# Skylarking/MARL

Hardware: AMD Instinct MI355X
Metric: env_steps_per_sec (higher is better)
Workload: dtype f32 (bf16x6 split products, fp32 accumulate)

## Files before the change

include/marl_hip.h:

```cpp
#ifndef MARL_HIP_H
#define MARL_HIP_H
#include <stddef.h>
#ifdef __cplusplus
extern "C" {
#endif

typedef struct {
  const float* p0; long ld0; int k0;
  const float* p1; long ld1; int k1;
  const int* idx; int nhot; int hot_w;
  int nid;
  const float* m0; long ldm0;
  long rpe0, bs0, off0;
  long rpei, bsi, offi;
  const int* emap0;
} marl_src_t;

typedef struct {
  int groups;
  long gs_x0, gs_x1, gs_w, gs_b, gs_y, gs_m0;
} marl_group_t;

typedef struct {
  const float *fc1_w, *fc1_b;
// ... 18 lines not shown
                          int N, int O, int A, int last_action, int reuse_network, int cu_budget,
                          float* gi_out, const float* gi_in, void* stream);
int marl_agent_unroll_reuse_supported(int B, int T, int N, int O, int A, int cu_budget);

typedef struct {
  float *w_ih, *w_hh;
  float *b_ih, *b_hh;
  float *fc2_w, *fc2_b;
} marl_agent_grads_t;

size_t marl_agent_bwd_workspace(int B, int N, int A);
int marl_agent_unroll_bwd(const marl_agent_weights_t* w, const float* dq, const int* dq_idx,
                          const float* dq_val, const int* dq_idx2, const float* dq_val2, int dq_gdiv, const float* dhs,
                          const float* saved, const float* hs, float* dxp, float* dh0,
                          const marl_agent_grads_t* g, float* ws, size_t ws_bytes,
                          int B, int T, int N, int A, void* stream);

int marl_q_gather(const float* q, const int* idx, const float* avail, float mask_val, float* out,
                  long rows, int A, void* stream);
int marl_q_masked_max(const float* q, const float* avail, float mask_val, float* out_max, int* out_arg,
                      long rows, int A, void* stream);
int marl_q_double_select(const float* q_sel, const float* q_val, const float* avail, float mask_val,
                         float* out_val, int* out_arg, long rows, int A, void* stream);
int marl_q_scatter(float* dq, const int* idx1, const float* g1, const int* idx2, const float* g2,
                   long rows, int A, int gdiv, void* stream);
int marl_vec_add(const float* a, const float* b, float* out, long n, void* stream);
int marl_agent_sum(const float* in, long ld_in, float* out, long ld_out, long rows, int N, int D, void* stream);
int marl_agent_bcast(const float* in, long ld_in, float* out, long ld_out, long rows, int N, int D, int accumulate,
                     void* stream);

int marl_qmix_mix_fwd(const float* hy, long ldh, const float* b2, const float* w22, const float* b22, const float* q,
                      float* q_tot, long rows, int N, int E, void* stream);
int marl_qmix_mix_bwd(const float* hy, long ldh, const float* q, const float* dq_tot, const float* w22, float* dhy,
                      float* db2, float* dq, long rows, int N, int E, void* stream);
int marl_qmix_tail_fwd(const marl_src_t* s, long rows, int S, const float* Wb1, long ldb1, const float* bb1, const float* Wh,
                       long ldwh, const float* bh, float* hy, long ldhy, int c_b1, int c_h, void* stream);

typedef struct {
  const float *w1, *w1_b;
  const float *b1, *b1_b;
  const float *w2, *w2_b;
  const float *h, *h_b;
  const float *b2_w, *b2_b;
} marl_qmix_weights_t;
int marl_qmix_fused_supported(int N, int S, int E);
size_t marl_qmix_fused_workspace(long rows, int N, int S);
// ... 261 lines not shown
```

marl_amd/_lib.py:

```python
from __future__ import annotations

import ctypes as C
import os

_HERE = os.path.dirname(os.path.abspath(__file__))
LIB_PATH = os.environ.get("MARL_HIP_LIB") or os.path.join(_HERE, "libmarl_hip.so")

c_float_p = C.c_void_p
c_int_p = C.c_void_p


class MarlSrc(C.Structure):
    _fields_ = [("p0", C.c_void_p), ("ld0", C.c_long), ("k0", C.c_int),
                ("p1", C.c_void_p), ("ld1", C.c_long), ("k1", C.c_int),
                ("idx", C.c_void_p), ("nhot", C.c_int), ("hot_w", C.c_int),
                ("nid", C.c_int),
                ("m0", C.c_void_p), ("ldm0", C.c_long),
                ("rpe0", C.c_long), ("bs0", C.c_long), ("off0", C.c_long),
                ("rpei", C.c_long), ("bsi", C.c_long), ("offi", C.c_long),
                ("emap0", C.c_void_p)]


class MarlGroup(C.Structure):
    _fields_ = [("groups", C.c_int), ("gs_x0", C.c_long), ("gs_x1", C.c_long), ("gs_w", C.c_long),
# ... 67 lines not shown
WW, WG = C.POINTER(MarlWorldWeights), C.POINTER(MarlWorldGrads)
MW, MG = C.POINTER(MarlMaicWeights), C.POINTER(MarlMaicGrads)
MIW, MIG = C.POINTER(MarlMaicInfer), C.POINTER(MarlMaicInferGrads)

SIGNATURES = {
    "marl_linear": (I, [SRC, P, L, I, P, P, L, I, I, I, I, F, GRP, P]),
    "marl_linear_wgrad": (I, [P, L, P, L, SRC, P, L, P, I, I, I, I, GRP, P, SZ, P]),
    "marl_linear_wgrad_workspace": (SZ, [I, I, I, I]),
    "marl_wgrad_slabs": (I, [I]),
    "marl_agent_unroll_fwd": (I, [AW, P, L, I, P, L, I, P, P, P, P, P, P, P, I, I, I, I, I, I, I, I, P, P, P]),
    "marl_agent_unroll_reuse_supported": (I, [I, I, I, I, I, I]),
    "marl_agent_unroll_x6_supported": (I, [I, I, I, I, I, I, I]),
    "marl_agent_unroll_x6_plain_r6": (I, [I, I, I, I, I, I, I, I]),
    "marl_agent_unroll_fwd_x6": (I, [AW, P, L, I, P, L, I, P, P, P, P, P, P, P, I, I, I, I, I, I, I, I, P, P, P]),
    "marl_agent_bwd_workspace": (SZ, [I, I, I]),
    "marl_agent_unroll_bwd_x6_supported": (I, [I, I, I, I, I]),
    "marl_agent_bwd_x6_workspace": (SZ, [I, I, I]),
    "marl_agent_unroll_bwd_x6": (I, [AW, P, P, P, P, I, P, P, P, P, AG, P, SZ, I, I, I, I, P]),
    "marl_agent_unroll_bwd": (I, [AW, P, P, P, P, P, I, P, P, P, P, P, AG, P, SZ, I, I, I, I, P]),
    "marl_replay_gather": (I, [P, I, I, I, I] + [P] * 17 + [P]),
    "marl_q_gather": (I, [P, P, P, F, P, L, I, P]),
    "marl_q_masked_max": (I, [P, P, F, P, P, L, I, P]),
    "marl_q_double_select": (I, [P, P, P, F, P, P, L, I, P]),
    "marl_q_scatter": (I, [P, P, P, P, P, L, I, I, P]),
    "marl_vec_add": (I, [P, P, P, L, P]),
    "marl_agent_sum": (I, [P, L, P, L, L, I, I, P]),
    "marl_agent_bcast": (I, [P, L, P, L, L, I, I, I, P]),
    "marl_qmix_mix_fwd": (I, [P, L, P, P, P, P, P, L, I, I, P]),
    "marl_qmix_mix_bwd": (I, [P, L, P, P, P, P, P, P, L, I, I, P]),
    "marl_qmix_tail_fwd": (I, [SRC, L, I, P, L, P, P, L, P, P, L, I, I, P]),
    "marl_qmix_fused_supported": (I, [I, I, I]),
    "marl_qmix_fused_workspace": (SZ, [L, I, I]),
    "marl_qmix_fused_fwd": (I, [QW, SRC, P, P, L, I, I, I, P]),
    "marl_qmix_fused_bwd": (I, [QW, SRC, P, P, P, QW, P, SZ, L, I, I, I, P]),
    "marl_qmix_fused_loss_bwd": (I, [QW, SRC, P, P, P, P, P, F, P, P, QW, P, P, SZ, L, I, I, I, P]),
    "marl_qmix_fused_fwd_x6": (I, [QW, SRC, P, P, L, I, I, I, P]),
    "marl_qmix_fused_bwd_x6": (I, [QW, SRC, P, P, P, QW, P, SZ, L, I, I, I, P]),
    "marl_qmix_fused_loss_bwd_x6": (I, [QW, SRC, P, P, P, P, P, F, P, P, QW, P, P, SZ, L, I, I, I, P]),
    "marl_qmix_wide_supported": (I, [I, I, I]),
    "marl_qmix_wide_workspace": (SZ, [L, I, I, I]),
    "marl_qmix_wide_fwd_kernel": (C.c_char_p, [L, I, I, I]),
    "marl_qmix_wide_fwd": (I, [QW, SRC, P, P, P, SZ, L, I, I, I, I, P]),
    "marl_qmix_wide_bwd": (I, [QW, SRC, P, P, P, QW, P, SZ, L, I, I, I, I, P]),
    "marl_qmix_wide_loss_bwd": (I, [QW, SRC, P, P, P, P, P, F, P, P, QW, P, P, SZ, L, I, I, I, I, P]),
    "marl_mlp3_supported": (I, [SRC, I, I, I, I, I]),
    "marl_mlp3_fwd": (I, [M3, SRC, P, L, L, L, I, I, I, P]),
# ... 96 lines not shown
```

marl_amd/algorithm/common.py:

```python
from __future__ import annotations

import copy
import numbers
import os
import warnings
import weakref

import numpy as np
import torch

from .. import ops, experiments
from ..hostutil import FlatParams, DeviceBatch, AsyncInt, require_cuda
from ..network.mixer import x6_mode
from ..rollout import EpisodeBatch

MASK_BIG = -9999999.0
MASK_QTRAN_EVAL = -999999.0
N_STATS = 4


class FlatView:

    def __init__(self, flat, params, start):
        self.params = list(params)
# ... 142 lines not shown
        self._td_dbg = {}
        self.max_episode_len = args.episode_limit
        self.gamma = args.gamma
        self.lr = args.lr
        self.model_dir = args.model_dir + '/' + args.alg + '/' + args.map
        self.args = args
        self.device = require_cuda(name)

        self.eval_net = mac
        self.eval_net.cuda()
        self.target_net = copy.deepcopy(mac)

    def _ready(self, needs_avail):
        args = self.args
        self.optimizer = FusedOptimizer(self._flat, args.optimizer, self.lr, args.grad_norm_clip)
        self._buf = Scratch()
        self.reducer = GradReducer()
        self.pair = PairedUnroll(x6=x6_mode(args))
        self.loss_readback = LossReadback(args)
        self.graphs = GraphedUpdate.from_args(args) if self.replay_graphs else None
        self.needs_avail = needs_avail
        self.last_stats = None
        self.sync_replicas()

    def _update_targets(self):
        self.target_net.agent._flat.flat.copy_(self.eval_net.agent._flat.flat)
        if self.mixer is not None and self.mixer._flat.n:
            self.target_mixer._flat.flat.copy_(self.mixer._flat.flat)

    def _g(self, name, shape, dt=torch.float32):
        return self._buf.get(name, shape, self.device, dt)

    def _td_inputs(self, db, q_next_tot):
        lam = self.td_lambda = td_lambda_of(self.args)
        if lam is None:
            self._td_dbg = {}
            return db.r, self.gamma
        G = self._g("td_ret", (db.B * db.T,))
        ops.td_lambda_returns(q_next_tot, db.r, db.term, db.padded, self.gamma, lam, G, db.B, db.T)
        self._td_dbg = {"td_targets": G}
        return G, 0.0

    def get_max_episode_len(self, batch):
        T = DeviceBatch.first_terminated_len(torch.as_tensor(np.asarray(batch['terminated'])), self.args.episode_limit)
        for key in batch.keys():
            batch[key] = batch[key][:, :T]
# ... 8 lines not shown
            self._full_len_streak = self._full_len_streak + 1 if full else 0
            return db
        db, pending = DeviceBatch.from_record_begin(rec, self.args, reducer=self.reducer, index=index, small=small)
        self.max_episode_len = db.T
        self._forward_backward(db)
        T = pending()
        if T == db.T:
            return None
        self._full_len_streak = 0
        return DeviceBatch.from_record(rec, self.args, T=T, index=index, small=small)

    def train(self, batch, train_step):
        ring = batch.ring if isinstance(batch, EpisodeBatch) else None
        if self.graphs is not None and ring is not None and self.graphs.run(self, ring, batch.index):
            db = None
        elif isinstance(batch, DeviceBatch):
            db = batch
        elif ring is not None:
            prep = self.graphs.prepared if self.graphs is not None else None
            if prep is not None:
                self.graphs.prepared = None
                db = DeviceBatch.from_record(ring, self.args, T=prep[1], index=batch.index, small=prep[0])
            else:
                small = ring.select_small(batch.index, avail_cur=self.needs_avail)
                db = self._device_batch(ring, batch.index, small)
        elif isinstance(batch, EpisodeBatch) and batch.record is not None:
            db = self._device_batch(batch.record, None, None)
        else:
            T = None
            if self.reducer.enabled:
                T = DeviceBatch.first_terminated_len(torch.as_tensor(np.asarray(batch['terminated'])),
                                                     self.args.episode_limit, reducer=self.reducer)
            db = DeviceBatch.from_dict(batch, self.args, self.device, T=T)
        if db is not None:
            self.max_episode_len = db.T
            self._forward_backward(db)
        return self._finish_update(train_step)

    def _loss_fn(self):
        return lambda s: s[0] / s[1]

    def _finish_update(self, train_step):
        self.reducer.allreduce_(self._flat.gradx)
        stats = self._flat.stats
        self.optimizer.step(den=stats[self.den_slot:self.den_slot + 1])
        if train_step > 0 and train_step % self.args.target_update_cycle == 0:
            self._update_targets()
# ... 182 lines not shown
    SCHEDULE_ARGS = ("gemm_mode", "mixer_dtype", "mixer_wgrad_dtype", "double_q", "no_loss_fold", "lazy_loss", "gamma",
                     "two_hyper_layers", "last_action", "reuse_network", "td_lambda")

    @staticmethod
    def _schedule_key(args):
        return (experiments.generation,) + tuple(repr(getattr(args, k, None)) for k in GraphedUpdate.SCHEDULE_ARGS)

    def run(self, learner, ring, index):
        self.prepared = None
        if self.disabled:
            return False
        args = learner.args
        if self.auto and int(index.numel()) > self.AUTO_MAX_EPISODES:
            return False
        if ring.T != args.episode_limit or int(index.numel()) != int(args.batch_size):
            return False
        key = (id(ring), int(index.numel()), ring.T)
        e = self.entries.get(key)
        if e is not None and e["ring"]() is not ring:
            e = None
        dev = ring.obs.device
        if e is None:
            idx = index.to(device=dev, dtype=torch.long).clone()
            small = ring.select_small(idx, avail_cur=getattr(learner, "needs_avail", False))
            db = DeviceBatch.from_record(ring, args, T=min(ring.T, args.episode_limit), index=idx, small=small)
            fused = getattr(small, "avail_next", None) is not None and db.T == ring.T
            e = self.entries[key] = dict(ring=weakref.ref(ring), idx=idx, small=small, db=db, calls=0, graph=None, streak=0,
                                         fused=fused, avail_next=None if fused else db.avail_next.clone(),
                                         u_act=None if fused else db.u_act.clone())
            if not fused:
                db.avail_next, db.u_act = e["avail_next"], e["u_act"]
            e["T"] = db.T
        idx, small, db = e["idx"], e["small"], e["db"]
        idx.copy_(index)
        db.o_map.copy_(idx)
        ring.select_small(idx, out=small)
        if e["graph"] is not None and (e["ws_gen"] != ops.WS.gen or e["sched_key"] != self._schedule_key(args)):
            e["graph"], e["ws_keep"], e["calls"] = None, None, 0
        pending = None
        term = small.term
        if e["graph"] is not None and e["streak"] >= 2 and term.is_cuda and term.dtype == torch.float32 and term.shape[0] > 0:
            out = ops.first_terminated_len(term, args.episode_limit)
            r = learner.reducer
            if r is not None and r.enabled:
                r.dist.all_reduce(out, op=r.dist.ReduceOp.MAX, group=r.group)
            pending = AsyncInt(out)
            T = e["T"]
        else:
            T = DeviceBatch.first_terminated_len(term, args.episode_limit, reducer=learner.reducer)
# ... 42 lines not shown
```

marl_amd/algorithm/q_learner.py:

```python
from __future__ import annotations

import copy

import numpy as np
import torch

from .. import ops, experiments
from ..hostutil import flatten_module
from ..network.mixer import VDNMixer, QMixMixer, DMAQer
from .common import MASK_BIG, LearnerParams, FlatView, Learner, agent_backward


class QLearner(Learner):
    def __init__(self, mac, args):
        self._begin(mac, args, "QLearner")
        if args.alg == 'vdn':
            self.mixer = VDNMixer(args)
        elif args.alg == 'qmix':
            self.mixer = QMixMixer(args)
        elif args.alg == 'qplex':
            self.mixer = DMAQer(args)
        else:
            raise ValueError("Mixer {} not recognised.".format(args.alg))
        self.target_mixer = copy.deepcopy(self.mixer)
# ... 30 lines not shown
        if keep_hs:
            hs, hs_tgt = g("hs", (B, T, N, H)), g("hs_tgt", (B, T, N, H))
            hs_en = g("hs_en", (B, T, N, H)) if a.double_q else None
        (oc, oc_bs, oc_t0), (on, on_bs, on_t0) = db.o_cur, db.o_next

        emap = getattr(db, 'o_map', None)
        cont, gi = None, None
        if a.double_q:
            shifted = on is oc and on_bs == oc_bs and on_t0 == oc_t0 + 1
            split = self.pair.chain_split(B * N, T, a.obs_shape)
            if shifted and ((self.eval_net.unroll_x6(B, T, oc) and experiments.get("fwd_xs") != 0) or
                            ops.agent_unroll_reuse_supported(B, T, N, a.obs_shape, A, split[0] if split else 256)):
                gi = g("gi", ops.saved_shape(T, B, N, planes=3))
            cont = lambda cu: self.eval_net.unroll(on, on_bs, on_t0, db.u_fed, db.u_bs, 0, B, T, q_en, hs_en, h_scr, None, h0=h_last,
                                                   ep_len=db.ep_len, ep_map=emap, cu_budget=cu, gi_in=gi)
        self.pair.run_chain(B * N, T, a.obs_shape,
                            lambda cu: self.eval_net.unroll(oc, oc_bs, oc_t0, db.u_fed, db.u_bs, -1, B, T, q_evals, hs, h_last, saved,
                                                            h0=None, ep_len=db.ep_len, ep_map=emap, cu_budget=cu, gi_out=gi),
                            cont,
                            lambda cu: self.target_net.unroll(on, on_bs, on_t0, db.u_fed, db.u_bs, 0, B, T, q_tgt, hs_tgt, None, None,
                                                              h0=None, ep_len=db.ep_len, ep_map=emap, cu_budget=cu))
        return q_evals, q_en, q_tgt, saved, (hs, hs_en, hs_tgt)

    def _select(self, db, q_evals, q_en, q_tgt):
        R, A, g = db.B * db.T * db.N, db.A, self._g
        q_chosen, q_tgt_chosen = g("q_chosen", (R,)), g("q_tgt_chosen", (R,))
        ops.q_gather(q_evals, db.u_act.reshape(-1), q_chosen, R, A)
        cur_max = None
        if self.args.double_q:
            cur_max = g("cur_max", (R,), torch.int32)
            ops.q_double_select(q_en, q_tgt, db.avail_next, MASK_BIG, q_tgt_chosen, cur_max, R, A)
        else:
            ops.q_masked_max(q_tgt, db.avail_next, MASK_BIG, q_tgt_chosen, None, R, A)
        return q_chosen, q_tgt_chosen, cur_max

    def _mix(self, db, q_evals, q_tgt, q_chosen, q_tgt_chosen, cur_max):
        a, g = self.args, self._g
        N, BT, A = db.N, db.B * db.T, db.A
        R = BT * N
        ctx, fold = {}, False
        qc, qtc = q_chosen.view(BT, N), q_tgt_chosen.view(BT, N)
        if a.alg == 'qplex':
            max_q = g("max_q", (R,))
            ops.q_masked_max(q_evals, db.avail, MASK_BIG, max_q, None, R, A)
            v_tot, a_tot = self.mixer.hip_forward(qc, db.s, BT, u_idx=db.u_taken.reshape(-1), max_q=max_q.view(BT, N), ctx=ctx)
            q_tot = g("q_tot", (BT,))
            ops.vec_add(v_tot, a_tot, q_tot, BT)
            if a.double_q:
                tgt_max = g("tgt_max", (R,))
                ops.q_masked_max(q_tgt, db.avail_next, MASK_BIG, tgt_max, None, R, A)
                vt, at = self.target_mixer.hip_forward(qtc, db.s_next, BT, u_idx=cur_max, max_q=tgt_max.view(BT, N), tag="t")
                q_tot_tgt = g("q_tot_tgt", (BT,))
                ops.vec_add(vt, at, q_tot_tgt, BT)
            else:
# ... 51 lines not shown
```

marl_amd/csrc/mixers.hip:

```cpp
#include "common.h"
#include "sums.h"
#include "../../include/marl_hip.h"

namespace {

constexpr int TPB = 256;
static_assert(TPB == SUMS_TPB, "the loss kernels launch sums.h's workgroup size");
inline int nblk(long n, int cap = 65535 * 16) {
  long b = (n + TPB - 1) / TPB;
  if (b > cap) b = cap;
  if (b < 1) b = 1;
  return (int)b;
}

__global__ void q_gather_kernel(const float* q, const int* idx, const float* avail, float mask_val, float* out,
                                long rows, int A) {
  for (long r = (long)blockIdx.x * TPB + threadIdx.x; r < rows; r += (long)gridDim.x * TPB) {
    const int a = idx[r];
    float v = 0.f;
    if (a >= 0) v = (avail && avail[r * A + a] == 0.f) ? mask_val : q[r * A + a];
    out[r] = v;
  }
}

__global__ void q_masked_max_kernel(const float* q, const float* avail, float mask_val, float* out_max,
                                    int* out_arg, long rows, int A) {
  for (long r = (long)blockIdx.x * TPB + threadIdx.x; r < rows; r += (long)gridDim.x * TPB) {
    float best = 0.f;
    int arg = 0;
    for (int a = 0; a < A; ++a) {
      float v = q[r * A + a];
      if (avail && avail[r * A + a] == 0.f) v = mask_val;
      if (a == 0 || v > best) { best = v; arg = a; }
    }
    if (out_max) out_max[r] = best;
    if (out_arg) out_arg[r] = arg;
  }
}

constexpr int DS_ROWS = 64;
__global__ __launch_bounds__(256) void q_double_select_kernel(const float* q_sel, const float* q_val, const float* avail,
                                                              float mask_val, float* out_val, int* out_arg, long rows, int A, int vec) {
  extern __shared__ __attribute__((aligned(16))) float ds_smem[];
  const int lane = threadIdx.x & 63, wave = threadIdx.x >> 6;
  const int TS = (DS_ROWS * A + 3) & ~3;
  float* Sq = ds_smem + (size_t)wave * 3 * TS;
  float* Sv = Sq + TS;
  float* Sa = Sv + TS;
  const long tiles = (rows + DS_ROWS - 1) / DS_ROWS;
  for (long tile = (long)blockIdx.x * 4 + wave; tile < tiles; tile += (long)gridDim.x * 4) {
    const long r0 = tile * DS_ROWS;
    const int n = (int)((rows - r0 < DS_ROWS ? rows - r0 : DS_ROWS) * A);
    const float* gq = q_sel + r0 * A;
    const float* gv = q_val + r0 * A;
    const float* ga = avail ? avail + r0 * A : nullptr;
    const int n4 = vec ? n >> 2 : 0;
    for (int e = lane; e < n4; e += 64) {
      reinterpret_cast<f32x4*>(Sq)[e] = reinterpret_cast<const f32x4*>(gq)[e];
      reinterpret_cast<f32x4*>(Sv)[e] = reinterpret_cast<const f32x4*>(gv)[e];
      reinterpret_cast<f32x4*>(Sa)[e] = ga ? reinterpret_cast<const f32x4*>(ga)[e] : (f32x4){1.f, 1.f, 1.f, 1.f};
    }
    for (int e = 4 * n4 + lane; e < n; e += 64) {
      Sq[e] = gq[e]; Sv[e] = gv[e]; Sa[e] = ga ? ga[e] : 1.f;
    }
    __builtin_amdgcn_s_waitcnt(0xC07F);
    const long r = r0 + lane;
    if (r < rows) {
      float best = 0.f; int arg = 0;
      for (int a = 0; a < A; ++a) {
        float v = Sq[lane * A + a];
        if (Sa[lane * A + a] == 0.f) v = mask_val;
        if (a == 0 || v > best) { best = v; arg = a; }
      }
      out_val[r] = Sa[lane * A + arg] == 0.f ? mask_val : Sv[lane * A + arg];
      if (out_arg) out_arg[r] = arg;
    }
  }
}

__global__ void q_double_select_rows_kernel(const float* q_sel, const float* q_val, const float* avail, float mask_val,
                                            float* out_val, int* out_arg, long rows, int A) {
  for (long r = (long)blockIdx.x * TPB + threadIdx.x; r < rows; r += (long)gridDim.x * TPB) {
    float best = 0.f;
    int arg = 0;
    for (int a = 0; a < A; ++a) {
      float v = q_sel[r * A + a];
      if (avail && avail[r * A + a] == 0.f) v = mask_val;
      if (a == 0 || v > best) { best = v; arg = a; }
    }
    out_val[r] = (avail && avail[r * A + arg] == 0.f) ? mask_val : q_val[r * A + arg];
    if (out_arg) out_arg[r] = arg;
  }
}

__global__ __launch_bounds__(256) void q_masked_max_tiled_kernel(const float* q, const float* avail, float mask_val, float* out_max,
                                                                 int* out_arg, long rows, int A) {
  extern __shared__ __attribute__((aligned(16))) float ds_smem[];
  const int lane = threadIdx.x & 63, wave = threadIdx.x >> 6;
  const int TS = (DS_ROWS * A + 3) & ~3;
  float* Sq = ds_smem + (size_t)wave * 2 * TS;
  float* Sa = Sq + TS;
  const long tiles = (rows + DS_ROWS - 1) / DS_ROWS;
  for (long tile = (long)blockIdx.x * 4 + wave; tile < tiles; tile += (long)gridDim.x * 4) {
    const long r0 = tile * DS_ROWS;
    const int n = (int)((rows - r0 < DS_ROWS ? rows - r0 : DS_ROWS) * A);
    const float* gq = q + r0 * A;
    const float* ga = avail ? avail + r0 * A : nullptr;
    const int n4 = n >> 2;
    for (int e = lane; e < n4; e += 64) {
      reinterpret_cast<f32x4*>(Sq)[e] = reinterpret_cast<const f32x4*>(gq)[e];
      reinterpret_cast<f32x4*>(Sa)[e] = ga ? reinterpret_cast<const f32x4*>(ga)[e] : (f32x4){1.f, 1.f, 1.f, 1.f};
    }
    for (int e = 4 * n4 + lane; e < n; e += 64) { Sq[e] = gq[e]; Sa[e] = ga ? ga[e] : 1.f; }
// ... 370 lines not shown
  MARL_CHECK_LAUNCH();
  return 0;
}

extern "C" int marl_q_masked_max(const float* q, const float* avail, float mask_val, float* out_max, int* out_arg,
                                 long rows, int A, void* stream) {
  if (rows <= 0) return 0;
  const size_t lds = (size_t)4 * 2 * ((DS_ROWS * A + 3) & ~3) * sizeof(float);
  if (((reinterpret_cast<uintptr_t>(q) | reinterpret_cast<uintptr_t>(avail)) & 15) == 0 && lds <= 64 * 1024 && rows >= 4096) {
    const long tiles = (rows + DS_ROWS - 1) / DS_ROWS;
    long nb = (tiles + 3) / 4;
    if (nb > 2048) nb = 2048;
    hipLaunchKernelGGL(q_masked_max_tiled_kernel, dim3((unsigned)nb), dim3(256), lds, (hipStream_t)stream, q, avail, mask_val,
                       out_max, out_arg, rows, A);
    MARL_CHECK_LAUNCH();
    return 0;
  }
  hipLaunchKernelGGL(q_masked_max_kernel, dim3(nblk(rows)), dim3(TPB), 0, (hipStream_t)stream, q, avail, mask_val,
                     out_max, out_arg, rows, A);
  MARL_CHECK_LAUNCH();
  return 0;
}

extern "C" int marl_q_double_select(const float* q_sel, const float* q_val, const float* avail, float mask_val,
                                    float* out_val, int* out_arg, long rows, int A, void* stream) {
  if (rows <= 0) return 0;
  const long tiles = (rows + DS_ROWS - 1) / DS_ROWS;
  long nb = (tiles + 3) / 4;
  if (nb > 2048) nb = 2048;
  const size_t lds = (size_t)4 * 3 * ((DS_ROWS * A + 3) & ~3) * sizeof(float);
  if (lds > 64 * 1024) {
    hipLaunchKernelGGL(q_double_select_rows_kernel, dim3(nblk(rows)), dim3(TPB), 0, (hipStream_t)stream, q_sel, q_val, avail,
                       mask_val, out_val, out_arg, rows, A);
    MARL_CHECK_LAUNCH();
    return 0;
  }
  const int vec = ((reinterpret_cast<uintptr_t>(q_sel) | reinterpret_cast<uintptr_t>(q_val) | reinterpret_cast<uintptr_t>(avail)) & 15) == 0;
  hipLaunchKernelGGL(q_double_select_kernel, dim3((unsigned)nb), dim3(256), lds, (hipStream_t)stream, q_sel, q_val, avail,
                     mask_val, out_val, out_arg, rows, A, vec);
  MARL_CHECK_LAUNCH();
  return 0;
}

extern "C" int marl_q_scatter(float* dq, const int* idx1, const float* g1, const int* idx2, const float* g2,
                              long rows, int A, int gdiv, void* stream) {
  if (rows <= 0) return 0;
  hipLaunchKernelGGL(q_scatter_kernel, dim3(nblk(rows)), dim3(TPB), 0, (hipStream_t)stream, dq, idx1, g1, idx2, g2,
                     rows, A, gdiv < 1 ? 1 : gdiv);
  MARL_CHECK_LAUNCH();
  return 0;
}

extern "C" int marl_vec_add(const float* a, const float* b, float* out, long n, void* stream) {
  if (n <= 0) return 0;
  hipLaunchKernelGGL(vec_add_kernel, dim3(nblk(n, 4096)), dim3(TPB), 0, (hipStream_t)stream, a, b, out, n);
  MARL_CHECK_LAUNCH();
  return 0;
}

extern "C" int marl_agent_sum(const float* in, long ld_in, float* out, long ld_out, long rows, int N, int D, void* stream) {
  if (rows <= 0) return 0;
  if (ld_in < D || ld_out < D) return (int)hipErrorInvalidValue;
  hipLaunchKernelGGL(agent_sum_kernel, dim3(nblk(rows * D)), dim3(TPB), 0, (hipStream_t)stream, in, ld_in, out, ld_out, rows, N, D);
  MARL_CHECK_LAUNCH();
// ... 101 lines not shown
  hipError_t e = hipMemsetAsync(out, 0, sizeof(int), s);
  if (e != hipSuccess) return (int)e;
  if (E <= 0 || T <= 0) return 0;
  long nb = ((long)E * 64 + TPB - 1) / TPB; if (nb > 256) nb = 256;
  hipLaunchKernelGGL(first_term_kernel, dim3((unsigned)nb), dim3(TPB), 0, s, term, ld, E, T, out);
  MARL_CHECK_LAUNCH();
  return 0;
}

namespace {
struct GatherArgs {
  const long long* idx;
  const int *u_src, *length_src, *won_src;
  const float *r_src, *term_src, *padded_src, *avail_src;
  int *o_map, *u, *u_act, *length, *won;
  float *r, *term, *padded, *avail_next, *avail_cur;
  int B, T, N, A;
};
__global__ __launch_bounds__(TPB) void replay_gather_kernel(GatherArgs a) {
  const int b = blockIdx.x;
  const long e = (long)a.idx[b];
  const int TNA = a.T * a.N * a.A;
  const float* av = a.avail_src + (e * (a.T + 1) + 1) * (long)a.N * a.A;
  float* ao = a.avail_next + (long)b * TNA;
  for (int i = blockIdx.y * 1024 + threadIdx.x; i < TNA && i < (blockIdx.y + 1) * 1024; i += TPB) ao[i] = av[i];
  if (a.avail_cur) {
    const int NA = a.N * a.A;
    const long live = (long)a.length_src[e] * NA;
    const float* ac = av - NA;
    float* co = a.avail_cur + (long)b * TNA;
    for (int i = blockIdx.y * 1024 + threadIdx.x; i < TNA && i < (blockIdx.y + 1) * 1024; i += TPB) co[i] = i < live ? ac[i] : 0.f;
  }
  if (blockIdx.y != 0) return;
  const int TN = a.T * a.N;
  for (int i = threadIdx.x; i < TN; i += TPB) {
    const int v = a.u_src[e * TN + i];
    a.u[(long)b * TN + i] = v;
    a.u_act[(long)b * TN + i] = v < 0 ? 0 : v;
  }
  for (int i = threadIdx.x; i < a.T; i += TPB) {
    a.r[(long)b * a.T + i] = a.r_src[e * a.T + i];
    a.term[(long)b * a.T + i] = a.term_src[e * a.T + i];
    a.padded[(long)b * a.T + i] = a.padded_src[e * a.T + i];
  }
  if (threadIdx.x == 0) {
    a.o_map[b] = (int)e;
    a.length[b] = a.length_src[e];
    a.won[b] = a.won_src[e];
  }
}
}

extern "C" int marl_replay_gather(const long long* idx, int B, int T, int N, int A, const int* u_src, const float* r_src,
                                  const float* term_src, const float* padded_src, const int* length_src,
                                  const int* won_src, const float* avail_src, int* o_map, int* u, int* u_act, float* r,
                                  float* term, float* padded, int* length, int* won, float* avail_next, float* avail_cur,
                                  void* stream) {
  if (B <= 0 || T <= 0) return 0;
  GatherArgs a;
  a.idx = idx; a.u_src = u_src; a.length_src = length_src; a.won_src = won_src;
  a.r_src = r_src; a.term_src = term_src; a.padded_src = padded_src; a.avail_src = avail_src;
  a.o_map = o_map; a.u = u; a.u_act = u_act; a.length = length; a.won = won;
  a.r = r; a.term = term; a.padded = padded; a.avail_next = avail_next; a.avail_cur = avail_cur;
  a.B = B; a.T = T; a.N = N; a.A = A;
  const int chunks = (T * N * A + 1023) / 1024;
  hipLaunchKernelGGL(replay_gather_kernel, dim3((unsigned)B, (unsigned)(chunks > 0 ? chunks : 1)), dim3(TPB), 0, (hipStream_t)stream, a);
  MARL_CHECK_LAUNCH();
  return 0;
}

extern "C" size_t marl_loss_workspace(long rows) { return (size_t)1024 * 4 * sizeof(float); }

extern "C" int marl_td_loss(const float* q_tot, const float* q_tot_tgt, const float* r, const float* term,
                            const float* padded, float gamma, float* dq_tot, float* out2, float* ws, long rows,
                            void* stream) {
  if (rows <= 0) return 0;
  const int nb = loss_blocks(rows);
  hipLaunchKernelGGL(td_loss_kernel, dim3(nb), dim3(TPB), 0, (hipStream_t)stream, q_tot, q_tot_tgt, r, term, padded,
                     gamma, dq_tot, ws, rows);
  MARL_CHECK_LAUNCH();
  hipLaunchKernelGGL(finish_sums_kernel, dim3(1), dim3(TPB), 0, (hipStream_t)stream, (const float*)ws, nb, 2, out2);
  MARL_CHECK_LAUNCH();
  return 0;
}

extern "C" int marl_qtran_loss(const float* jq, const float* jq_tgt, const float* v, const float* jq_hat,
                               const float* qsum_opt, const float* qsum_nopt, const float* r, const float* term,
                               const float* padded, float gamma, float lam_opt, float lam_nopt, float* d_jq,
// ... 13 lines not shown
```

marl_amd/env/synthetic_smac.py:

```python
from __future__ import annotations

import torch

from .. import ops
from ..hostutil import require_cuda


class EpisodeRecord:

    def __init__(self, E, T, N, O, S, A, device):
        self.E, self.T, self.N, self.O, self.S, self.A = E, T, N, O, S, A
        z = lambda *s, dt=torch.float32: torch.zeros(*s, dtype=dt, device=device)
        self.obs, self.state_store, self.avail = z(E, T + 1, N, O), z(E, T + 1, (S + 3) // 4 * 4), z(E, T + 1, N, A)
        self.u = torch.full((E, T, N), -1, dtype=torch.int32, device=device)
        self.r, self.term, self.padded = z(E, T), z(E, T), z(E, T)
        self.length = z(E, dt=torch.int32)
        self.won = z(E, dt=torch.int32)

    FIELDS = ("obs", "state_store", "avail", "u", "r", "term", "padded", "length", "won")

    @property
    def state(self):
        return None if self.state_store is None else self.state_store[..., :self.S]

    def index_select(self, idx):
        out = EpisodeRecord.__new__(EpisodeRecord)
        out.E, out.T, out.N, out.O, out.S, out.A = int(idx.numel()), self.T, self.N, self.O, self.S, self.A
        for f in self.FIELDS:
            setattr(out, f, getattr(self, f).index_select(0, idx))
        return out

    def slice(self, i0, i1):
        out = EpisodeRecord.__new__(EpisodeRecord)
        out.E, out.T, out.N, out.O, out.S, out.A = i1 - i0, self.T, self.N, self.O, self.S, self.A
        for f in self.FIELDS:
            setattr(out, f, getattr(self, f)[i0:i1])
        return out

    def clone(self):
        out = EpisodeRecord.__new__(EpisodeRecord)
        out.E, out.T, out.N, out.O, out.S, out.A = self.E, self.T, self.N, self.O, self.S, self.A
        for f in self.FIELDS:
            setattr(out, f, getattr(self, f).clone())
        return out

    SMALL = ("avail", "u", "r", "term", "padded", "length", "won")

    def select_small(self, idx, out=None, avail_cur=False):
        B = int(idx.numel())
        if self.u.is_cuda:
            if out is None:
                out = EpisodeRecord.__new__(EpisodeRecord)
                out.E, out.T, out.N, out.O, out.S, out.A = B, self.T, self.N, self.O, self.S, self.A
                out.obs = out.state_store = out.avail = None
                dev = self.u.device
                mk = lambda *s, dt=torch.float32: torch.empty(*s, dtype=dt, device=dev)
                out.u, out.u_act = mk(B, self.T, self.N, dt=torch.int32), mk(B, self.T, self.N, dt=torch.int32)
                out.r, out.term, out.padded = mk(B, self.T), mk(B, self.T), mk(B, self.T)
                out.length, out.won, out.o_map = mk(B, dt=torch.int32), mk(B, dt=torch.int32), mk(B, dt=torch.int32)
                out.avail_next = mk(B, self.T, self.N, self.A)
                out.avail_cur = mk(B, self.T, self.N, self.A) if avail_cur else None
            ops.replay_gather(idx.to(torch.long).contiguous(), self, out)
            return out
        if out is not None:
            for f in self.SMALL:
                torch.index_select(getattr(self, f), 0, idx, out=getattr(out, f))
            return out
        out = EpisodeRecord.__new__(EpisodeRecord)
        out.E, out.T, out.N, out.O, out.S, out.A = B, self.T, self.N, self.O, self.S, self.A
        out.obs = out.state_store = None
        for f in self.SMALL:
            setattr(out, f, getattr(self, f).index_select(0, idx))
        return out

    def copy_into(self, dst, idx):
        for f in self.FIELDS:
            getattr(dst, f).index_copy_(0, idx, getattr(self, f))


class SyntheticSMACEnv:
    batched = True

    def __init__(self, n_envs, n_agents, obs_shape, state_shape, n_actions, episode_limit, seed=1, env0=0,
# ... 60 lines not shown
```

marl_amd/experiments.py:

```python
from __future__ import annotations

import contextlib
import os
import warnings

LIB_DEFAULTS = {"fwd_xs": 1, "fwd_w2l": 1, "bwd_pipe_max_rt": 4, "wgrad_tall": 1, "wide_res": 1, "rollout_v1": 0, "unroll_r6": 1}
HOST_DEFAULTS = {"no_pair": 0, "no_chain": 0, "chain_split": None, "mlp3_keep": 1, "x6_bwd_min_wg": 1, "force_reducer": 0}


def _env_int(name, default):
    v = os.environ.get("MARL_" + name.upper())
    if v is None or v == "":
        return default
    try:
        return int(v)
    except ValueError:
        warnings.warn("MARL_%s=%r ignored (want an integer)" % (name.upper(), v))
        return default


_lib_values = {k: _env_int(k, d) for k, d in LIB_DEFAULTS.items()}
_host_values = {k: _env_int(k, d) for k, d in HOST_DEFAULTS.items()}
if _host_values["chain_split"] is not None and not (_host_values["chain_split"] == 0 or
                                                      (8 <= _host_values["chain_split"] <= 248 and _host_values["chain_split"] % 8 == 0)):
    warnings.warn("MARL_CHAIN_SPLIT=%r ignored (want 0 or a multiple of 8 in 8..248)" % _host_values["chain_split"])
    _host_values["chain_split"] = None
_applied = None
generation = 0


# ... 44 lines not shown
```

marl_amd/hostutil.py:

```python
from __future__ import annotations

import numpy as np
import torch
import torch.nn as nn

from . import ops


def require_cuda(what="the MARL hot path"):
    if not torch.cuda.is_available():
        raise RuntimeError("%s runs only on the MI355X HIP kernels (no CPU fallback); "
                           "torch.cuda.is_available() is False" % what)
    return torch.device("cuda", torch.cuda.current_device())


class FlatParams:

    def __init__(self, params, device, with_grad=True):
        self.params = list(params)
        self.offsets = []
        off = 0
        for p in self.params:
            self.offsets.append(off)
            off += (p.numel() + 3) // 4 * 4
# ... 212 lines not shown
        self.o_map = None
        idx = None
        if index is not None:
            idx = index.to(device=rec.obs.device, dtype=torch.long)
            rec = small if small is not None else rec.select_small(idx)
            self.o_map = rec.o_map if getattr(rec, "o_map", None) is not None else idx.to(torch.int32).contiguous()
        E = rec.E
        if T is None:
            T = cls.first_terminated_len(rec.term, args.episode_limit)
        if T > Ta:
            raise ValueError("max_episode_len %d exceeds the %d steps the episode record holds "
                             "(args.episode_limit != record length?)" % (T, Ta))
        self.B, self.T, self.N, self.O, self.S, self.A = E, T, N, O, S, A
        self.o_cur = (big.obs, (Ta + 1) * N, 0)
        self.o_next = (big.obs, (Ta + 1) * N, 1)
        self.ep_len = rec.length
        st2 = big.state_store.view(big.E * (Ta + 1), -1)[:, :S]
        self.s = ops.Rows(st2, (T, Ta + 1, 0), self.o_map)
        self.s_next = ops.Rows(st2, (T, Ta + 1, 1), self.o_map)
        self.u_fed = rec.u
        self.u_bs = Ta * N
        cutc = lambda x: x[:, :T].contiguous()
        self.u_taken = cutc(rec.u)
        fused = getattr(rec, "avail_next", None) is not None
        self.u_act = cutc(rec.u_act) if fused else self.u_taken.clamp(min=0)
        self.r, self.term, self.padded = cutc(rec.r).view(-1), cutc(rec.term).view(-1), cutc(rec.padded).view(-1)
        if fused and getattr(rec, "avail_cur", None) is not None:
            self._avail = rec.avail_cur[:, :T].reshape(E * T * N, A)
        self._avail_src = (rec, T) if rec.avail is not None else (big, T, idx, rec.length)
        self.avail_next = (rec.avail_next[:, :T] if fused else rec.avail[:, 1:T + 1]).reshape(E * T * N, A)
        return self

    @property
    def avail(self):
        if "_avail" not in self.__dict__:
            if len(self._avail_src) == 2:
                rec, T = self._avail_src
                av, length = rec.avail[:, :T], rec.length
            else:
                big, T, idx, length = self._avail_src
                av = big.avail.index_select(0, idx)[:, :T]
            t_idx = torch.arange(T, device=av.device)[None, :, None, None]
            live = t_idx < length[:, None, None, None]
            self._avail = torch.where(live, av, torch.zeros((), device=av.device)).reshape(-1, av.shape[-1])
        return self._avail

    @avail.setter
    def avail(self, v):
        self._avail = v


def pin_to_gpu_numa(device_index=0):
    import glob
    import os
# ... 18 lines not shown
```

marl_amd/ops.py:

```python
from __future__ import annotations

import ctypes as C

import torch

from . import _lib
from ._lib import (MarlSrc, MarlGroup, MarlAgentWeights, MarlAgentGrads, MarlQmixWeights, MarlMlp3Weights,
                   MarlQtranWeights, MarlRtwWeights, MarlWorldWeights, MarlWorldGrads, MarlMaicWeights, MarlMaicGrads, MarlMaicInfer,
                   MarlMaicInferGrads, check)


def _p(t):
    return None if t is None else C.c_void_p(t.data_ptr())


def _stream():
    return C.c_void_p(torch.cuda.current_stream().cuda_stream)


def _f32(t):
    assert t.dtype == torch.float32 and t.is_cuda, "expected a CUDA float32 tensor"
    return t


# ... 196 lines not shown
        _i32(dq_idx2); _f32(dq_val2)
    check(lib.marl_agent_unroll_bwd(C.byref(w), _p(_f32(dq)) if dq is not None else None, _p(dq_idx), _p(dq_val),
                                    _p(dq_idx2), _p(dq_val2), int(dq_gdiv), _p(dhs),
                                    _p(_f32(saved)), _p(hs), _p(_f32(dxp)),
                                    _p(dh0), C.byref(g), _p(ws), ws.numel() * 4, B, T, N, A, _stream()),
          "marl_agent_unroll_bwd")


def q_gather(q, idx, out, rows, A, avail=None, mask_val=0.0):
    check(_lib.load().marl_q_gather(_p(_f32(q)), _p(_i32(idx)), _p(avail), float(mask_val), _p(_f32(out)), rows, A,
                                    _stream()), "marl_q_gather")


def q_masked_max(q, avail, mask_val, out_max, out_arg, rows, A):
    check(_lib.load().marl_q_masked_max(_p(_f32(q)), _p(avail), float(mask_val), _p(out_max), _p(out_arg), rows, A,
                                        _stream()), "marl_q_masked_max")


def q_double_select(q_sel, q_val, avail, mask_val, out_val, out_arg, rows, A):
    check(_lib.load().marl_q_double_select(_p(_f32(q_sel)), _p(_f32(q_val)), _p(avail), float(mask_val), _p(_f32(out_val)),
                                           _p(out_arg), rows, A, _stream()), "marl_q_double_select")


def q_scatter(dq, idx1, g1, idx2, g2, rows, A, gdiv=1):
    check(_lib.load().marl_q_scatter(_p(_f32(dq)), _p(idx1), _p(g1), _p(idx2), _p(g2), rows, A, gdiv, _stream()),
          "marl_q_scatter")


def vec_add(a, b, out, n):
    check(_lib.load().marl_vec_add(_p(_f32(a)), _p(_f32(b)), _p(_f32(out)), n, _stream()), "marl_vec_add")


def _ld(t, D):
    return t.stride(0) if (t.dim() == 2 and t.shape[1] == D and t.stride(1) == 1) else D


def agent_sum(inp, out, rows, N, D):
    check(_lib.load().marl_agent_sum(_p(_f32(inp)), _ld(inp, D), _p(_f32(out)), _ld(out, D), rows, N, D, _stream()),
          "marl_agent_sum")


def agent_bcast(inp, out, rows, N, D, accumulate=False):
    check(_lib.load().marl_agent_bcast(_p(_f32(inp)), _ld(inp, D), _p(_f32(out)), _ld(out, D), rows, N, D,
                                       1 if accumulate else 0, _stream()), "marl_agent_bcast")


# ... 20 lines not shown
          "marl_qmix_tail_fwd")


def qplex_mix_fwd(w_raw, v, q, max_q, key, ag, ac, v_tot, a_tot, lam_out, rows, N, K, weighted, minus_one):
    check(_lib.load().marl_qplex_mix_fwd(_p(w_raw), _p(v), _p(q), _p(max_q), _p(key), _p(ag), _p(ac), _p(v_tot),
                                         _p(a_tot), _p(lam_out), rows, N, K, int(weighted), int(minus_one), _stream()),
          "marl_qplex_mix_fwd")


def qplex_mix_bwd(w_raw, q, max_q, key, ag, ac, g, dq, dw_raw, dv, dkey, dag, dac, rows, N, K, weighted, minus_one):
    check(_lib.load().marl_qplex_mix_bwd(_p(w_raw), _p(q), _p(max_q), _p(key), _p(ag), _p(ac), _p(g), _p(dq),
                                         _p(dw_raw), _p(dv), _p(dkey), _p(dag), _p(dac), rows, N, K, int(weighted),
                                         int(minus_one), _stream()), "marl_qplex_mix_bwd")


_FT_OUT = {}


def replay_gather(idx, src, out):
    assert idx.dtype == torch.int64 and idx.is_cuda and idx.is_contiguous()
    B, T, N, A = int(idx.numel()), src.T, src.N, src.A
    for t in (src.u, src.r, src.term, src.padded, src.length, src.won, src.avail, out.u, out.u_act, out.r, out.term, out.padded,
              out.length, out.won, out.avail_next, out.o_map):
        assert t.is_cuda and t.is_contiguous()
    assert src.u.dtype == torch.int32 and src.length.dtype == torch.int32 and src.won.dtype == torch.int32
    check(_lib.load().marl_replay_gather(_p(idx), B, T, N, A, _p(src.u), _p(_f32(src.r)), _p(_f32(src.term)), _p(_f32(src.padded)),
                                         _p(src.length), _p(src.won), _p(_f32(src.avail)), _p(_i32(out.o_map)), _p(_i32(out.u)),
                                         _p(_i32(out.u_act)), _p(_f32(out.r)), _p(_f32(out.term)), _p(_f32(out.padded)),
                                         _p(_i32(out.length)), _p(_i32(out.won)), _p(_f32(out.avail_next)),
                                         _p(getattr(out, "avail_cur", None)), _stream()),
          "marl_replay_gather")


def first_terminated_len(term, T):
    t2 = term.reshape(term.shape[0], -1)
    assert t2.dtype == torch.float32 and t2.is_cuda and t2.stride(1) == 1
    ring = _FT_OUT.get(t2.device)
    if ring is None:
        ring = _FT_OUT[t2.device] = [torch.zeros(8, dtype=torch.int32, device=t2.device), 0]
    out = ring[0][ring[1] % 8:ring[1] % 8 + 1]
    ring[1] += 1
    check(_lib.load().marl_first_terminated_len(_p(t2), t2.stride(0), t2.shape[0], min(T, t2.shape[1]), _p(out), _stream()),
          "marl_first_terminated_len")
    return out


def td_loss(q_tot, q_tgt, r, term, padded, gamma, dq_tot, out2, rows):
    lib = _lib.load()
    ws = WS.get("loss", lib.marl_loss_workspace(rows), q_tot.device)
    check(lib.marl_td_loss(_p(_f32(q_tot)), _p(_f32(q_tgt)), _p(_f32(r)), _p(_f32(term)), _p(_f32(padded)),
                           float(gamma), _p(_f32(dq_tot)), _p(_f32(out2)), _p(ws), rows, _stream()), "marl_td_loss")

# ... 538 lines not shown
```

Measured before the change: 69.91 million.

## Read next-step avail masks directly from replay ring in double-Q select

Adds a ring-indexed variant of the double-Q select kernel that reads next-step availability masks straight from the replay buffer through the episode map, instead of reading a gathered copy. For QMIX with double_q (on by default via the select_fold flag), the replay gather no longer materialises avail_next, which removes one B*T*N*A copy per batch. avail_next becomes a lazily built property for consumers that still need it, and the gather kernel launches fewer chunks when no avail tensor is written. The cost is extra index arithmetic and scattered, less-aligned loads in the select kernel, and a lazy fallback copy if another path touches avail_next.

```diff
diff --git a/include/marl_hip.h b/include/marl_hip.h
--- a/include/marl_hip.h
+++ b/include/marl_hip.h
@@ -64,6 +64,8 @@
                       long rows, int A, void* stream);
 int marl_q_double_select(const float* q_sel, const float* q_val, const float* avail, float mask_val,
                          float* out_val, int* out_arg, long rows, int A, void* stream);
+int marl_q_double_select_ring(const float* q_sel, const float* q_val, const float* avail, const int* emap, long rpe, long bs,
+                              long off, int N, float mask_val, float* out_val, int* out_arg, long rows, int A, void* stream);
 int marl_q_scatter(float* dq, const int* idx1, const float* g1, const int* idx2, const float* g2,
                    long rows, int A, int gdiv, void* stream);
 int marl_vec_add(const float* a, const float* b, float* out, long n, void* stream);
diff --git a/marl_amd/_lib.py b/marl_amd/_lib.py
--- a/marl_amd/_lib.py
+++ b/marl_amd/_lib.py
@@ -113,6 +113,7 @@
     "marl_q_gather": (I, [P, P, P, F, P, L, I, P]),
     "marl_q_masked_max": (I, [P, P, F, P, P, L, I, P]),
     "marl_q_double_select": (I, [P, P, P, F, P, P, L, I, P]),
+    "marl_q_double_select_ring": (I, [P, P, P, P, L, L, L, I, F, P, P, L, I, P]),
     "marl_q_scatter": (I, [P, P, P, P, P, L, I, I, P]),
     "marl_vec_add": (I, [P, P, P, L, P]),
     "marl_agent_sum": (I, [P, L, P, L, L, I, I, P]),
diff --git a/marl_amd/algorithm/common.py b/marl_amd/algorithm/common.py
--- a/marl_amd/algorithm/common.py
+++ b/marl_amd/algorithm/common.py
@@ -188,6 +188,10 @@
         self.needs_avail = needs_avail
         self.last_stats = None
         self.sync_replicas()
+
+    def _wants_avail_next(self):
+        f = getattr(self, "wants_avail_next", None)
+        return True if f is None else bool(f())
 
     def _update_targets(self):
         self.target_net.agent._flat.flat.copy_(self.eval_net.agent._flat.flat)
@@ -242,7 +246,7 @@
                 self.graphs.prepared = None
                 db = DeviceBatch.from_record(ring, self.args, T=prep[1], index=batch.index, small=prep[0])
             else:
-                small = ring.select_small(batch.index, avail_cur=self.needs_avail)
+                small = ring.select_small(batch.index, avail_cur=self.needs_avail, avail_next=self._wants_avail_next())
                 db = self._device_batch(ring, batch.index, small)
         elif isinstance(batch, EpisodeBatch) and batch.record is not None:
             db = self._device_batch(batch.record, None, None)
@@ -471,9 +475,9 @@
         dev = ring.obs.device
         if e is None:
             idx = index.to(device=dev, dtype=torch.long).clone()
-            small = ring.select_small(idx, avail_cur=getattr(learner, "needs_avail", False))
+            small = ring.select_small(idx, avail_cur=getattr(learner, "needs_avail", False), avail_next=learner._wants_avail_next())
             db = DeviceBatch.from_record(ring, args, T=min(ring.T, args.episode_limit), index=idx, small=small)
-            fused = getattr(small, "avail_next", None) is not None and db.T == ring.T
+            fused = getattr(small, "u_act", None) is not None and db.T == ring.T
             e = self.entries[key] = dict(ring=weakref.ref(ring), idx=idx, small=small, db=db, calls=0, graph=None, streak=0,
                                          fused=fused, avail_next=None if fused else db.avail_next.clone(),
                                          u_act=None if fused else db.u_act.clone())
diff --git a/marl_amd/algorithm/q_learner.py b/marl_amd/algorithm/q_learner.py
--- a/marl_amd/algorithm/q_learner.py
+++ b/marl_amd/algorithm/q_learner.py
@@ -76,6 +76,13 @@
                                                               h0=None, ep_len=db.ep_len, ep_map=emap, cu_budget=cu))
         return q_evals, q_en, q_tgt, saved, (hs, hs_en, hs_tgt)
 
+    def _avail_in_place(self):
+        a = self.args
+        return a.alg == 'qmix' and bool(a.double_q) and experiments.get("select_fold") != 0 and not getattr(a, "no_loss_fold", False)
+
+    def wants_avail_next(self):
+        return not self._avail_in_place()
+
     def _select(self, db, q_evals, q_en, q_tgt):
         R, A, g = db.B * db.T * db.N, db.A, self._g
         q_chosen, q_tgt_chosen = g("q_chosen", (R,)), g("q_tgt_chosen", (R,))
@@ -83,7 +90,11 @@
         cur_max = None
         if self.args.double_q:
             cur_max = g("cur_max", (R,), torch.int32)
-            ops.q_double_select(q_en, q_tgt, db.avail_next, MASK_BIG, q_tgt_chosen, cur_max, R, A)
+            rows = getattr(db, "avail_next_rows", None) if self._avail_in_place() else None
+            if rows is not None:
+                ops.q_double_select_ring(q_en, q_tgt, rows, db.N, MASK_BIG, q_tgt_chosen, cur_max, R, A)
+            else:
+                ops.q_double_select(q_en, q_tgt, db.avail_next, MASK_BIG, q_tgt_chosen, cur_max, R, A)
         else:
             ops.q_masked_max(q_tgt, db.avail_next, MASK_BIG, q_tgt_chosen, None, R, A)
         return q_chosen, q_tgt_chosen, cur_max
diff --git a/marl_amd/csrc/mixers.hip b/marl_amd/csrc/mixers.hip
--- a/marl_amd/csrc/mixers.hip
+++ b/marl_amd/csrc/mixers.hip
@@ -39,8 +39,19 @@
 }
 
 constexpr int DS_ROWS = 64;
+typedef float f32x4u __attribute__((ext_vector_type(4), aligned(4)));
+struct RingAvail {
+  const int* emap;
+  long tna, sna, ona;
+  FastDiv fd;
+};
+__device__ __forceinline__ long ring_delta(const RingAvail& ra, unsigned b) {
+  return (long)(ra.emap ? ra.emap[b] : (int)b) * ra.sna + ra.ona - (long)b * ra.tna;
+}
+template <bool RING>
 __global__ __launch_bounds__(256) void q_double_select_kernel(const float* q_sel, const float* q_val, const float* avail,
-                                                              float mask_val, float* out_val, int* out_arg, long rows, int A, int vec) {
+                                                              float mask_val, float* out_val, int* out_arg, long rows, int A, int vec,
+                                                              RingAvail ra) {
   extern __shared__ __attribute__((aligned(16))) float ds_smem[];
   const int lane = threadIdx.x & 63, wave = threadIdx.x >> 6;
   const int TS = (DS_ROWS * A + 3) & ~3;
@@ -53,15 +64,43 @@
     const int n = (int)((rows - r0 < DS_ROWS ? rows - r0 : DS_ROWS) * A);
     const float* gq = q_sel + r0 * A;
     const float* gv = q_val + r0 * A;
-    const float* ga = avail ? avail + r0 * A : nullptr;
+    const float* ga = (avail && !RING) ? avail + r0 * A : nullptr;
     const int n4 = vec ? n >> 2 : 0;
     for (int e = lane; e < n4; e += 64) {
       reinterpret_cast<f32x4*>(Sq)[e] = reinterpret_cast<const f32x4*>(gq)[e];
       reinterpret_cast<f32x4*>(Sv)[e] = reinterpret_cast<const f32x4*>(gv)[e];
-      reinterpret_cast<f32x4*>(Sa)[e] = ga ? reinterpret_cast<const f32x4*>(ga)[e] : (f32x4){1.f, 1.f, 1.f, 1.f};
+      if (!RING) reinterpret_cast<f32x4*>(Sa)[e] = ga ? reinterpret_cast<const f32x4*>(ga)[e] : (f32x4){1.f, 1.f, 1.f, 1.f};
     }
     for (int e = 4 * n4 + lane; e < n; e += 64) {
-      Sq[e] = gq[e]; Sv[e] = gv[e]; Sa[e] = ga ? ga[e] : 1.f;
+      Sq[e] = gq[e]; Sv[e] = gv[e];
+      if (!RING) Sa[e] = ga ? ga[e] : 1.f;
+    }
+    if (RING) {
+      const unsigned f0 = (unsigned)(r0 * A);
+      const unsigned b0 = fastdiv(f0, ra.fd), b1 = fastdiv(f0 + (unsigned)n - 1u, ra.fd);
+      if (b1 - b0 <= 1u) {
+        const long d0 = ring_delta(ra, b0), d1 = ring_delta(ra, b1);
+        const unsigned fb = (b0 + 1u) * (unsigned)ra.tna;
+        const int n4r = n >> 2;
+        for (int e = lane; e < n4r; e += 64) {
+          const unsigned f = f0 + 4u * (unsigned)e;
+          if (f + 3u < fb || f >= fb) {
+            reinterpret_cast<f32x4*>(Sa)[e] = *reinterpret_cast<const f32x4u*>(avail + ((long)f + (f < fb ? d0 : d1)));
+          } else {
+#pragma unroll
+            for (unsigned j = 0; j < 4u; ++j) Sa[4 * e + j] = avail[(long)(f + j) + (f + j < fb ? d0 : d1)];
+          }
+        }
+        for (int e = 4 * n4r + lane; e < n; e += 64) {
+          const unsigned f = f0 + (unsigned)e;
+          Sa[e] = avail[(long)f + (f < fb ? d0 : d1)];
+        }
+      } else {
+        for (int e = lane; e < n; e += 64) {
+          const unsigned f = f0 + (unsigned)e;
+          Sa[e] = avail[(long)f + ring_delta(ra, fastdiv(f, ra.fd))];
+        }
+      }
     }
     __builtin_amdgcn_s_waitcnt(0xC07F);
     const long r = r0 + lane;
@@ -78,17 +117,19 @@
   }
 }
 
+template <bool RING>
 __global__ void q_double_select_rows_kernel(const float* q_sel, const float* q_val, const float* avail, float mask_val,
-                                            float* out_val, int* out_arg, long rows, int A) {
+                                            float* out_val, int* out_arg, long rows, int A, RingAvail ra) {
   for (long r = (long)blockIdx.x * TPB + threadIdx.x; r < rows; r += (long)gridDim.x * TPB) {
     float best = 0.f;
     int arg = 0;
+    const float* av = !avail ? nullptr : RING ? avail + r * A + ring_delta(ra, fastdiv((unsigned)(r * A), ra.fd)) : avail + r * A;
     for (int a = 0; a < A; ++a) {
       float v = q_sel[r * A + a];
-      if (avail && avail[r * A + a] == 0.f) v = mask_val;
+      if (av && av[a] == 0.f) v = mask_val;
       if (a == 0 || v > best) { best = v; arg = a; }
     }
-    out_val[r] = (avail && avail[r * A + arg] == 0.f) ? mask_val : q_val[r * A + arg];
+    out_val[r] = (av && av[arg] == 0.f) ? mask_val : q_val[r * A + arg];
     if (out_arg) out_arg[r] = arg;
   }
 }
@@ -505,24 +546,43 @@
   return 0;
 }
 
-extern "C" int marl_q_double_select(const float* q_sel, const float* q_val, const float* avail, float mask_val,
-                                    float* out_val, int* out_arg, long rows, int A, void* stream) {
+template <bool RING>
+static int q_double_select_launch(const float* q_sel, const float* q_val, const float* avail, float mask_val,
+                                  float* out_val, int* out_arg, long rows, int A, const RingAvail& ra, void* stream) {
   if (rows <= 0) return 0;
   const long tiles = (rows + DS_ROWS - 1) / DS_ROWS;
   long nb = (tiles + 3) / 4;
   if (nb > 2048) nb = 2048;
   const size_t lds = (size_t)4 * 3 * ((DS_ROWS * A + 3) & ~3) * sizeof(float);
   if (lds > 64 * 1024) {
-    hipLaunchKernelGGL(q_double_select_rows_kernel, dim3(nblk(rows)), dim3(TPB), 0, (hipStream_t)stream, q_sel, q_val, avail,
-                       mask_val, out_val, out_arg, rows, A);
+    hipLaunchKernelGGL(q_double_select_rows_kernel<RING>, dim3(nblk(rows)), dim3(TPB), 0, (hipStream_t)stream, q_sel, q_val, avail,
+                       mask_val, out_val, out_arg, rows, A, ra);
     MARL_CHECK_LAUNCH();
     return 0;
   }
-  const int vec = ((reinterpret_cast<uintptr_t>(q_sel) | reinterpret_cast<uintptr_t>(q_val) | reinterpret_cast<uintptr_t>(avail)) & 15) == 0;
-  hipLaunchKernelGGL(q_double_select_kernel, dim3((unsigned)nb), dim3(256), lds, (hipStream_t)stream, q_sel, q_val, avail,
-                     mask_val, out_val, out_arg, rows, A, vec);
-  MARL_CHECK_LAUNCH();
-  return 0;
+  const int vec = ((reinterpret_cast<uintptr_t>(q_sel) | reinterpret_cast<uintptr_t>(q_val) | (RING ? 0 : reinterpret_cast<uintptr_t>(avail))) & 15) == 0;
+  hipLaunchKernelGGL(q_double_select_kernel<RING>, dim3((unsigned)nb), dim3(256), lds, (hipStream_t)stream, q_sel, q_val, avail,
+                     mask_val, out_val, out_arg, rows, A, vec, ra);
+  MARL_CHECK_LAUNCH();
+  return 0;
+}
+
+extern "C" int marl_q_double_select(const float* q_sel, const float* q_val, const float* avail, float mask_val,
+                                    float* out_val, int* out_arg, long rows, int A, void* stream) {
+  RingAvail ra;
+  ra.emap = nullptr; ra.tna = ra.sna = 1; ra.ona = 0; ra.fd = make_fastdiv(1);
+  return q_double_select_launch<false>(q_sel, q_val, avail, mask_val, out_val, out_arg, rows, A, ra, stream);
+}
+
+extern "C" int marl_q_double_select_ring(const float* q_sel, const float* q_val, const float* avail, const int* emap, long rpe,
+                                         long bs, long off, int N, float mask_val, float* out_val, int* out_arg, long rows,
+                                         int A, void* stream) {
+  if (rows <= 0) return 0;
+  if (!q_sel || !q_val || !avail || !out_val || A < 1 || N < 1 || rpe < 1 || off < 0 || bs < rpe + off || rows % N) return (int)hipErrorInvalidValue;
+  if (rows * A >= (1l << 31) || rpe * N * A >= (1l << 31)) return (int)hipErrorInvalidValue;
+  RingAvail ra;
+  ra.emap = emap; ra.tna = rpe * N * A; ra.sna = bs * N * A; ra.ona = off * N * A; ra.fd = make_fastdiv((unsigned)ra.tna);
+  return q_double_select_launch<true>(q_sel, q_val, avail, mask_val, out_val, out_arg, rows, A, ra, stream);
 }
 
 extern "C" int marl_q_scatter(float* dq, const int* idx1, const float* g1, const int* idx2, const float* g2,
@@ -670,8 +730,10 @@
   const long e = (long)a.idx[b];
   const int TNA = a.T * a.N * a.A;
   const float* av = a.avail_src + (e * (a.T + 1) + 1) * (long)a.N * a.A;
-  float* ao = a.avail_next + (long)b * TNA;
-  for (int i = blockIdx.y * 1024 + threadIdx.x; i < TNA && i < (blockIdx.y + 1) * 1024; i += TPB) ao[i] = av[i];
+  if (a.avail_next) {
+    float* ao = a.avail_next + (long)b * TNA;
+    for (int i = blockIdx.y * 1024 + threadIdx.x; i < TNA && i < (blockIdx.y + 1) * 1024; i += TPB) ao[i] = av[i];
+  }
   if (a.avail_cur) {
     const int NA = a.N * a.A;
     const long live = (long)a.length_src[e] * NA;
@@ -711,7 +773,7 @@
   a.o_map = o_map; a.u = u; a.u_act = u_act; a.length = length; a.won = won;
   a.r = r; a.term = term; a.padded = padded; a.avail_next = avail_next; a.avail_cur = avail_cur;
   a.B = B; a.T = T; a.N = N; a.A = A;
-  const int chunks = (T * N * A + 1023) / 1024;
+  const int chunks = (avail_next || avail_cur) ? (T * N * A + 1023) / 1024 : 1;
   hipLaunchKernelGGL(replay_gather_kernel, dim3((unsigned)B, (unsigned)(chunks > 0 ? chunks : 1)), dim3(TPB), 0, (hipStream_t)stream, a);
   MARL_CHECK_LAUNCH();
   return 0;
diff --git a/marl_amd/env/synthetic_smac.py b/marl_amd/env/synthetic_smac.py
--- a/marl_amd/env/synthetic_smac.py
+++ b/marl_amd/env/synthetic_smac.py
@@ -46,7 +46,7 @@
 
     SMALL = ("avail", "u", "r", "term", "padded", "length", "won")
 
-    def select_small(self, idx, out=None, avail_cur=False):
+    def select_small(self, idx, out=None, avail_cur=False, avail_next=True):
         B = int(idx.numel())
         if self.u.is_cuda:
             if out is None:
@@ -58,7 +58,7 @@
                 out.u, out.u_act = mk(B, self.T, self.N, dt=torch.int32), mk(B, self.T, self.N, dt=torch.int32)
                 out.r, out.term, out.padded = mk(B, self.T), mk(B, self.T), mk(B, self.T)
                 out.length, out.won, out.o_map = mk(B, dt=torch.int32), mk(B, dt=torch.int32), mk(B, dt=torch.int32)
-                out.avail_next = mk(B, self.T, self.N, self.A)
+                out.avail_next = mk(B, self.T, self.N, self.A) if avail_next else None
                 out.avail_cur = mk(B, self.T, self.N, self.A) if avail_cur else None
             ops.replay_gather(idx.to(torch.long).contiguous(), self, out)
             return out
diff --git a/marl_amd/experiments.py b/marl_amd/experiments.py
--- a/marl_amd/experiments.py
+++ b/marl_amd/experiments.py
@@ -5,7 +5,7 @@
 import warnings
 
 LIB_DEFAULTS = {"fwd_xs": 1, "fwd_w2l": 1, "bwd_pipe_max_rt": 4, "wgrad_tall": 1, "wide_res": 1, "rollout_v1": 0, "unroll_r6": 1}
-HOST_DEFAULTS = {"no_pair": 0, "no_chain": 0, "chain_split": None, "mlp3_keep": 1, "x6_bwd_min_wg": 1, "force_reducer": 0}
+HOST_DEFAULTS = {"no_pair": 0, "no_chain": 0, "chain_split": None, "mlp3_keep": 1, "x6_bwd_min_wg": 1, "force_reducer": 0, "select_fold": 1}
 
 
 def _env_int(name, default):
diff --git a/marl_amd/hostutil.py b/marl_amd/hostutil.py
--- a/marl_amd/hostutil.py
+++ b/marl_amd/hostutil.py
@@ -258,14 +258,30 @@
         self.u_bs = Ta * N
         cutc = lambda x: x[:, :T].contiguous()
         self.u_taken = cutc(rec.u)
-        fused = getattr(rec, "avail_next", None) is not None
+        fused = getattr(rec, "u_act", None) is not None
         self.u_act = cutc(rec.u_act) if fused else self.u_taken.clamp(min=0)
         self.r, self.term, self.padded = cutc(rec.r).view(-1), cutc(rec.term).view(-1), cutc(rec.padded).view(-1)
         if fused and getattr(rec, "avail_cur", None) is not None:
             self._avail = rec.avail_cur[:, :T].reshape(E * T * N, A)
         self._avail_src = (rec, T) if rec.avail is not None else (big, T, idx, rec.length)
-        self.avail_next = (rec.avail_next[:, :T] if fused else rec.avail[:, 1:T + 1]).reshape(E * T * N, A)
+        self.avail_next_rows = ops.Rows(big.avail.view(big.E * (Ta + 1), N * A), (T, Ta + 1, 1), self.o_map) \
+            if big.avail.is_contiguous() else None
+        if fused and rec.avail_next is None:
+            self._avail_next_src = (big, T, idx)
+        else:
+            self._avail_next = (rec.avail_next[:, :T] if fused else rec.avail[:, 1:T + 1]).reshape(E * T * N, A)
         return self
+
+    @property
+    def avail_next(self):
+        if "_avail_next" not in self.__dict__:
+            big, T, idx = self._avail_next_src
+            self._avail_next = big.avail.index_select(0, idx)[:, 1:T + 1].reshape(-1, big.A)
+        return self._avail_next
+
+    @avail_next.setter
+    def avail_next(self, v):
+        self._avail_next = v
 
     @property
     def avail(self):
diff --git a/marl_amd/ops.py b/marl_amd/ops.py
--- a/marl_amd/ops.py
+++ b/marl_amd/ops.py
@@ -242,6 +242,15 @@
                                            _p(out_arg), rows, A, _stream()), "marl_q_double_select")
 
 
+def q_double_select_ring(q_sel, q_val, avail, N, mask_val, out_val, out_arg, rows, A):
+    t = _f32(avail.t)
+    assert t.dim() == 2 and t.is_contiguous() and t.shape[1] == N * A
+    rpe, bs, off = avail.remap
+    check(_lib.load().marl_q_double_select_ring(_p(_f32(q_sel)), _p(_f32(q_val)), _p(t), _p(None if avail.emap is None else _i32(avail.emap)),
+                                                rpe, bs, off, N, float(mask_val), _p(_f32(out_val)), _p(out_arg), rows, A, _stream()),
+          "marl_q_double_select_ring")
+
+
 def q_scatter(dq, idx1, g1, idx2, g2, rows, A, gdiv=1):
     check(_lib.load().marl_q_scatter(_p(_f32(dq)), _p(idx1), _p(g1), _p(idx2), _p(g2), rows, A, gdiv, _stream()),
           "marl_q_scatter")
@@ -308,12 +317,12 @@
     B, T, N, A = int(idx.numel()), src.T, src.N, src.A
     for t in (src.u, src.r, src.term, src.padded, src.length, src.won, src.avail, out.u, out.u_act, out.r, out.term, out.padded,
               out.length, out.won, out.avail_next, out.o_map):
-        assert t.is_cuda and t.is_contiguous()
+        assert t is out.avail_next and t is None or t.is_cuda and t.is_contiguous()
     assert src.u.dtype == torch.int32 and src.length.dtype == torch.int32 and src.won.dtype == torch.int32
     check(_lib.load().marl_replay_gather(_p(idx), B, T, N, A, _p(src.u), _p(_f32(src.r)), _p(_f32(src.term)), _p(_f32(src.padded)),
                                          _p(src.length), _p(src.won), _p(_f32(src.avail)), _p(_i32(out.o_map)), _p(_i32(out.u)),
                                          _p(_i32(out.u_act)), _p(_f32(out.r)), _p(_f32(out.term)), _p(_f32(out.padded)),
-                                         _p(_i32(out.length)), _p(_i32(out.won)), _p(_f32(out.avail_next)),
+                                         _p(_i32(out.length)), _p(_i32(out.won)), _p(out.avail_next),
                                          _p(getattr(out, "avail_cur", None)), _stream()),
           "marl_replay_gather")
 
```

Result: no change. 69.88 million (median of 2 runs) (-0.0%).
